# jwliao1209/DiffMusic

Hardware: AMD Instinct MI355X
Metric: denoising steps/sec (10 s clip, 200-step DPS) (higher is better)
Workload: dtype f16; 1 GPU; MusicLDM + DPS music_inpainting, 10 s @16 kHz, 200-step schedule, batch 8 per GPU (BASELINE.json configs[1]); global_batch=8, clips_per_gpu=8, lanes=1, parallelism=clip-sharded x1 (RCCL world size 1, no per-step collective), finite=True, nan_steps=0, settle_steps=10, cached_reference_transform=True, launched_by=single process

## Files before the change

diffmusic_amd/csrc/elementwise.hip:

```cpp
#include "dmx_common.h"
#include <cstdlib>
#include "kernels.h"

namespace {

__device__ __forceinline__ void unpack8(const uint4& u, float* f) {
  f[0] = alo(u.x); f[1] = ahi(u.x); f[2] = alo(u.y); f[3] = ahi(u.y);
  f[4] = alo(u.z); f[5] = ahi(u.z); f[6] = alo(u.w); f[7] = ahi(u.w);
}
__device__ __forceinline__ uint4 pack8(const float* f) {
  return make_uint4(pack2a(f[0], f[1]), pack2a(f[2], f[3]), pack2a(f[4], f[5]), pack2a(f[6], f[7]));
}
__device__ __forceinline__ float silu_f(float z) { return z / (1.f + __expf(-z)); }
__device__ __forceinline__ float dsilu_f(float z) {
  const float s = 1.f / (1.f + __expf(-z));
  return s * (1.f + z * (1.f - s));
}

template <int MODE>
__global__ void gn_partial_kernel(const act_t* __restrict__ x, const act_t* __restrict__ dy,
                                  const float* __restrict__ scale, const float* __restrict__ shift,
                                  const float* __restrict__ stats, float* __restrict__ partial,
                                  int P, int C, int G, int rpb, int ppb, int silu) {
  extern __shared__ float sh[];
// ... 967 lines not shown
}

__global__ void gather_col_f32_kernel(const float* __restrict__ x, float* __restrict__ y, long long rows, int ld, int col) {
  const long long idx = (long long)blockIdx.x * blockDim.x + threadIdx.x;
  if (idx < rows) y[idx] = x[idx * ld + col];
}
__global__ void tanh_bwd_pad8_kernel(const float* __restrict__ dwav, const float* __restrict__ wav8, act_t* __restrict__ gz,
                                     long long rows) {
  const long long idx = (long long)blockIdx.x * blockDim.x + threadIdx.x;
  if (idx >= rows) return;
  const float w = wav8[idx * 8];
  const float g = dwav[idx] * (1.f - w * w);
  reinterpret_cast<uint4*>(gz)[idx] = make_uint4((uint32_t)f2a(g), 0u, 0u, 0u);
}
__global__ void gather_col_f32_dead_kernel(const float* __restrict__ x, float* __restrict__ y, long long rows, int ld, int col, int T, int s0,
                                           int s1) {
  const long long idx = (long long)blockIdx.x * blockDim.x + threadIdx.x;
  if (idx >= rows) return;
  const int t = (int)(idx % T);
  y[idx] = (t >= s0 && t < s1) ? 0.f : x[idx * ld + col];
}
__global__ void tanh_bwd_pad8_dead_kernel(const float* __restrict__ dwav, const float* __restrict__ wav8, act_t* __restrict__ gz,
                                          long long rows, int T, int s0, int s1) {
  const long long idx = (long long)blockIdx.x * blockDim.x + threadIdx.x;
  if (idx >= rows) return;
  const int t = (int)(idx % T);
  float g = 0.f;
  if (!(t >= s0 && t < s1)) {
    const float w = wav8[idx * 8];
    g = dwav[idx] * (1.f - w * w);
  }
  reinterpret_cast<uint4*>(gz)[idx] = make_uint4((uint32_t)f2a(g), 0u, 0u, 0u);
}
__global__ void scatter_col_pad8_kernel(const float* __restrict__ v, act_t* __restrict__ y, long long rows, float scale) {
  const long long idx = (long long)blockIdx.x * blockDim.x + threadIdx.x;
  if (idx >= rows) return;
  reinterpret_cast<uint4*>(y)[idx] = make_uint4((uint32_t)f2a(v[idx] * scale), 0u, 0u, 0u);
}

__global__ void gather_col_f32_to_act_kernel(const float* __restrict__ x, act_t* __restrict__ y, long long rows, int ld, int col) {
  const long long idx = (long long)blockIdx.x * blockDim.x + threadIdx.x;
  if (idx < rows) y[idx] = f2a(x[idx * ld + col]);
}
__global__ void pad_col8_act_kernel(const act_t* __restrict__ v, act_t* __restrict__ y, long long rows) {
  const long long idx = (long long)blockIdx.x * blockDim.x + threadIdx.x;
  if (idx >= rows) return;
  reinterpret_cast<uint4*>(y)[idx] = make_uint4((uint32_t)v[idx], 0u, 0u, 0u);
}

constexpr int GN_SMALL_MAXU = 16;
__global__ __launch_bounds__(256) void gn_small_kernel(const act_t* __restrict__ x, act_t* __restrict__ y,
                                                       const float* __restrict__ gamma, const float* __restrict__ beta,
                                                       float* __restrict__ stats, float* __restrict__ scale, float* __restrict__ shift,
                                                       int P, int C, int G, float eps, int silu) {
  __shared__ float sh[16];
  const int g = blockIdx.x, b = blockIdx.y, cpg = C / G, U = cpg >> 2, c0 = g * cpg;
  const int units = P * U;
  const act_t* xb = x + (long long)b * P * C + c0;
  uint2 v[GN_SMALL_MAXU];
  float sum = 0.f;
#pragma unroll
  for (int i = 0; i < GN_SMALL_MAXU; ++i) {
    const int u = threadIdx.x + i * 256;
    v[i] = make_uint2(0, 0);
    if (u < units) {
      const int px = u / U, cu = u - px * U;
// ... 247 lines not shown
  hipLaunchKernelGGL(bf16_to_f32_kernel, dim3((unsigned)((n + 255) / 256)), dim3(256), 0, st, x, y, n, scale);
  return CHECK_LAUNCH();
}
int dmx_extract_col(const act_t* x, float* y, long long rows, int ld, int col, hipStream_t st) {
  hipLaunchKernelGGL(extract_col_kernel, dim3((unsigned)((rows + 255) / 256)), dim3(256), 0, st, x, y, rows, ld, col);
  return CHECK_LAUNCH();
}
int dmx_timestep_embed(const float* t, act_t* y, int B, int dim, hipStream_t st) {
  hipLaunchKernelGGL(timestep_embed_kernel, dim3(cdiv(B * dim, 256)), dim3(256), 0, st, t, y, B, dim);
  return CHECK_LAUNCH();
}

int dmx_gather_col_f32(const float* x, float* y, long long rows, int ld, int col, hipStream_t st) {
  hipLaunchKernelGGL(gather_col_f32_kernel, dim3((unsigned)((rows + 255) / 256)), dim3(256), 0, st, x, y, rows, ld, col);
  return CHECK_LAUNCH();
}
int dmx_tanh_bwd_pad8(const float* dwav, const float* wav8, act_t* gz, long long rows, hipStream_t st) {
  hipLaunchKernelGGL(tanh_bwd_pad8_kernel, dim3((unsigned)((rows + 255) / 256)), dim3(256), 0, st, dwav, wav8, gz, rows);
  return CHECK_LAUNCH();
}
int dmx_scatter_col_pad8(const float* v, act_t* y, long long rows, float scale, hipStream_t st) {
  hipLaunchKernelGGL(scatter_col_pad8_kernel, dim3((unsigned)((rows + 255) / 256)), dim3(256), 0, st, v, y, rows, scale);
  return CHECK_LAUNCH();
}

int dmx_gather_col_f32_dead(const float* x, float* y, long long rows, int ld, int col, int T, int s0, int s1, hipStream_t st) {
  hipLaunchKernelGGL(gather_col_f32_dead_kernel, dim3((unsigned)((rows + 255) / 256)), dim3(256), 0, st, x, y, rows, ld, col, T, s0, s1);
  return CHECK_LAUNCH();
}
int dmx_tanh_bwd_pad8_dead(const float* dwav, const float* wav8, act_t* gz, long long rows, int T, int s0, int s1, hipStream_t st) {
  hipLaunchKernelGGL(tanh_bwd_pad8_dead_kernel, dim3((unsigned)((rows + 255) / 256)), dim3(256), 0, st, dwav, wav8, gz, rows, T, s0, s1);
  return CHECK_LAUNCH();
}
int dmx_gather_col_f32_to_act(const float* x, act_t* y, long long rows, int ld, int col, hipStream_t st) {
  hipLaunchKernelGGL(gather_col_f32_to_act_kernel, dim3((unsigned)((rows + 255) / 256)), dim3(256), 0, st, x, y, rows, ld, col);
  return CHECK_LAUNCH();
}
int dmx_pad_col8_act(const act_t* v, act_t* y, long long rows, hipStream_t st) {
  hipLaunchKernelGGL(pad_col8_act_kernel, dim3((unsigned)((rows + 255) / 256)), dim3(256), 0, st, v, y, rows);
  return CHECK_LAUNCH();
}
```

diffmusic_amd/csrc/hifigan.hip:

```cpp
#include "models.h"
#include "conv_pair.h"
#include <cstdlib>

struct SplitKScope {
  explicit SplitKScope(float* ws, size_t bytes, bool on) : on_(on && ws) { if (on_) dmx_gemm_set_splitk_workspace(ws, bytes); }
  ~SplitKScope() { if (on_) dmx_gemm_set_splitk_workspace(nullptr, 0); }
  bool on_;
};

struct Span { int a = 0, b = 0; bool empty() const { return b <= a; } };
static inline Span span_meet(Span x, Span y) { Span r{x.a > y.a ? x.a : y.a, x.b < y.b ? x.b : y.b}; if (r.empty()) r = Span{}; return r; }
static inline long long floor_div(long long a, long long b) { return a >= 0 ? a / b : -((-a + b - 1) / b); }
static inline long long ceil_div(long long a, long long b) { return -floor_div(-a, b); }

int dmx_conv_dead_rows_impl(int k, int dil, int pad, int stride, int transposed, int t_in, int t_out, int a, int b, int* lo, int* hi) {
  *lo = *hi = 0;
  if (k < 1 || dil < 1 || stride < 1 || pad < 0 || t_in < 1 || t_out < 1) return DMX_ERR_SHAPE;
  if (!transposed && stride != 1) return DMX_ERR_SHAPE;
  if (a < 0) a = 0;
  if (b > t_out) b = t_out;
  if (b <= a) return DMX_OK;
  const long long INF = 1ll << 40;
  const long long ea = a == 0 ? -INF : a, eb = b == t_out ? INF : b;
  long long l, h;
// ... 195 lines not shown

  int out_len(int T_) const {
    int t = T_;
    for (int i = 0; i < ns; ++i) t = conv_out_len(ups[i], t);
    return t;
  }

  int forward(const act_t* mel, float* wav, int B_, int T_, void* ws, size_t ws_bytes, hipStream_t st, int s0 = 0, int s1 = 0) {
    if (cfg.model_in_dim & 7) return DMX_ERR_SHAPE;
    dry = (ws == nullptr);
    B = B_;
    if (!dry) {
      use_dead = false;
      if (s1 > s0) { make_plan(T_, s0, s1); use_dead = plan.on; }
    }
    const bool dead = use_dead && !dry;
    SplitKScope sk_scope(splitk_ws, kSplitKBytes, !dry && !multi_wanted());
    arena.reset(ws, dry ? (size_t)-1 : ws_bytes);
    T = T_;
    Ts.assign(ns, 0);
    xs_a.assign(ns, nullptr); act_out.assign(ns, nullptr);
    ha.assign(ns * nk * nd, nullptr); xa.assign(ns * nk * nd, nullptr);
    hb.assign(ns * nk * nd, nullptr); xb.assign(ns * nk * nd, nullptr);
    fused.assign(ns * nk * nd, 0);
    const float slope = cfg.leaky_relu_slope;
    auto bits = [&](size_t rows, int C) { return (unsigned char*)arena.raw(rows * (size_t)(C >> 3)); };
    act_pre = arena.bf((size_t)B * T * conv_pre.Cop);
    {
      Epi e; e.flags = EPI_LRELU2 | EPI_NO_C; e.act_slope = slope; e.C2 = act_pre;
      RUN(conv_fwd_1d(conv_pre, mel, act_pre, B, T, e, st));
    }
    const act_t* cur_act = act_pre;
    int Tin = T;
    for (int s = 0; s < ns; ++s) {
      const ConvLayer& up = ups[s];
      const int To = conv_out_len(up, Tin), C = up.Cop;
      const size_t n = (size_t)B * To * C;
      Ts[s] = To;
      xs_a[s] = arena.bf(n);
      act_out[s] = arena.bf(n);
      unsigned char* xs_b = nullptr;
      for (int k = 0; k < nk; ++k)
        for (int d = 0; d < nd; ++d) {
          const int id = idx(s, k, d);
          fused[id] = step_is_fused(id, To) ? 1 : 0;
          xa[id] = d == 0 ? xs_a[s] : arena.bf(n);
          if (fused[id]) {
            hb[id] = bits((size_t)B * To, C);
            if (d == 0) { if (!xs_b) xs_b = bits((size_t)B * To, C); xb[id] = xs_b; }
            else xb[id] = bits((size_t)B * To, C);
          } else {
            ha[id] = arena.bf(n);
          }
        }
      const size_t mk = arena.mark();
      act_t* sum = arena.bf(n);
      {
        Epi e; e.flags = EPI_LRELU2 | EPI_NO_C; e.act_slope = slope; e.C2 = xs_a[s];
        if (xs_b) { e.flags |= EPI_BITS2; e.B2 = xs_b; }
        RUN(conv_fwd_1d(up, cur_act, xs_a[s], B, Tin, e, st));
      }
      const float next_slope = (s == ns - 1) ? 0.01f : slope;
      const bool mt = multi();
      bool all_fused = nk <= 3;
      for (int k = 0; k < nk; ++k) for (int d = 0; d < nd; ++d) all_fused = all_fused && fused[idx(s, k, d)] != 0;
      if (all_fused && !mt) {
        for (int d = 0; d < nd; ++d) {
          GemmDesc da[DMX_MAX_STAGES], db[DMX_MAX_STAGES];
          const GemmDesc* pa[DMX_MAX_STAGES]; const GemmDesc* pb[DMX_MAX_STAGES];
          PairDead pd[DMX_MAX_STAGES];
          for (int k = 0; k < nk; ++k) {
            const int id = idx(s, k, d);
            if (dead) pd[k] = dead_fwd(id);
            {
              Epi e; e.flags = EPI_LRELU2 | EPI_NO_C | EPI_BITS2; e.act_slope = slope; e.B2 = hb[id];
              RUN(conv_fwd_1d_desc(c1[id], xa[id], ha[id], B, To, e, da[k]));
            }
            if (d < nd - 1) {
              const int idn = idx(s, k, d + 1);
              act_t* xn = xa[idn];
              Epi e; e.flags = EPI_RESID | EPI_RESID_INV | EPI_LRELU2 | EPI_NO_C | EPI_BITS2; e.R = xa[id]; e.resid_inv_slope = 1.f / slope;
              e.act_slope = slope; e.C2 = xn; e.B2 = xb[idn];
              RUN(conv_fwd_1d_desc(c2[id], ha[id], xn, B, To, e, db[k]));
            } else {
              Epi e; e.flags = EPI_RESID | EPI_RESID_INV; e.R = xa[id]; e.resid_inv_slope = 1.f / slope; e.alpha = 1.f / nk;
              if (k > 0) e.flags |= EPI_ACCUM;
              if (k == nk - 1) { e.flags |= EPI_LRELU2 | EPI_NO_C; e.act_slope = next_slope; e.C2 = act_out[s]; }
              RUN(conv_fwd_1d_desc(c2[id], ha[id], sum, B, To, e, db[k]));
            }
            pa[k] = &da[k]; pb[k] = &db[k];
          }
          if (dry) continue;
          for (int k = 0; k < nk; ++k)
            if (!dmx_conv_pair_eligible(&da[k], db[k])) {
              dmx_set_error("hifigan: resblock step %d was planned as fused but the pair kernel refuses it", idx(s, k, d));
              return DMX_ERR_STATE;
            }
          if (d < nd - 1) RUN(dmx_conv_pair_group_launch(nk, pa, pb, st, dead ? pd : nullptr));
          else for (int k = 0; k < nk; ++k) RUN(conv_pair_run(da[k], db[k], st, dead ? &pd[k] : nullptr));
        }
        arena.release(mk);
        cur_act = act_out[s];
        Tin = To;
        continue;
      }
      hipEvent_t fin_prev = nullptr;
      if (mt) {
        hipEvent_t e0 = next_event();
        (void)hipEventRecord(e0, st);
        for (int k = 1; k < nk; ++k) (void)hipStreamWaitEvent(bstream[k], e0, 0);
      }
      for (int k = 0; k < nk; ++k) {
        hipStream_t sk = (mt && k > 0) ? bstream[k] : st;
        for (int d = 0; d < nd; ++d) {
          const int id = idx(s, k, d);
          const bool fz = fused[id] != 0;
          GemmDesc da, db;
          {
            Epi e; e.flags = EPI_LRELU2 | EPI_NO_C; e.act_slope = slope;
            if (fz) { e.flags |= EPI_BITS2; e.B2 = hb[id]; } else e.C2 = ha[id];
            RUN(conv_fwd_1d_desc(c1[id], xa[id], ha[id], B, To, e, da));
          }
          if (d < nd - 1) {
            const int idn = idx(s, k, d + 1);
            act_t* xn = xa[idn];
            Epi e; e.flags = EPI_RESID | EPI_RESID_INV | EPI_LRELU2 | EPI_NO_C; e.R = xa[id]; e.resid_inv_slope = 1.f / slope;
            e.act_slope = slope; e.C2 = xn;
            if (fused[idn]) { e.flags |= EPI_BITS2; e.B2 = xb[idn]; }
            RUN(conv_fwd_1d_desc(c2[id], ha[id], xn, B, To, e, db));
          } else {
            Epi e; e.flags = EPI_RESID | EPI_RESID_INV; e.R = xa[id]; e.resid_inv_slope = 1.f / slope; e.alpha = 1.f / nk;
            if (k > 0) e.flags |= EPI_ACCUM;
            if (k == nk - 1) { e.flags |= EPI_LRELU2 | EPI_NO_C; e.act_slope = next_slope; e.C2 = act_out[s]; }
            RUN(conv_fwd_1d_desc(c2[id], ha[id], sum, B, To, e, db));
          }
          if (!dry && fz && !dmx_conv_pair_eligible(&da, db)) {
            dmx_set_error("hifigan: resblock step %d was planned as fused but the pair kernel refuses it", id);
            return DMX_ERR_STATE;
          }
          if (d == nd - 1 && mt && fin_prev) (void)hipStreamWaitEvent(sk, fin_prev, 0);
          RUN(conv_pair_run(da, db, sk));
          if (d == nd - 1 && mt) { fin_prev = next_event(); (void)hipEventRecord(fin_prev, sk); }
        }
      }
      if (mt && fin_prev) (void)hipStreamWaitEvent(st, fin_prev, 0);
      arena.release(mk);
      cur_act = act_out[s];
      Tin = To;
    }
    const int Tout = Tin;
    wav8 = arena.f32((size_t)B * Tout * 8);
    CHECK_WS("hifigan");
    {
      Epi e; e.flags = EPI_F32OUT | EPI_TANH;
      RUN(conv_fwd_1d(conv_post, cur_act, wav8, B, Tout, e, st));
    }
    if (dead) RUN(dmx_gather_col_f32_dead(wav8, wav, (long long)B * Tout, 8, 0, Tout, plan.wav.a, plan.wav.b, st));
    else RUN(dmx_gather_col_f32(wav8, wav, (long long)B * Tout, 8, 0, st));
    have_tape = true;
    return DMX_OK;
  }

  int backward(const float* dwav, act_t* dmel, hipStream_t st) {
    if (!have_tape && !dry) { dmx_set_error("hifigan backward without forward"); return DMX_ERR_STATE; }
    SplitKScope sk_scope(splitk_ws, kSplitKBytes, !dry && !multi_wanted());
    const float slope = cfg.leaky_relu_slope;
    const int Tout = Ts[ns - 1];
    const size_t mk0 = arena.mark();
    act_t* gz = arena.bf((size_t)B * Tout * 8);
    const int Clast = ups[ns - 1].Cop;
    act_t* g = arena.bf((size_t)B * Tout * Clast);
    CHECK_WS("hifigan");
    const bool dead = use_dead && !dry;
    if (dead) RUN(dmx_tanh_bwd_pad8_dead(dwav, wav8, gz, (long long)B * Tout, Tout, plan.wav.a, plan.wav.b, st));
    else RUN(dmx_tanh_bwd_pad8(dwav, wav8, gz, (long long)B * Tout, st));
    {
      Epi e; e.flags = EPI_MASK; e.X = act_out[ns - 1]; e.mask_slope = 0.01f; e.alpha = 1.f / nk;
      RUN(conv_bwd_1d(conv_post, gz, g, B, Tout, e, st));
    }
    for (int s = ns - 1; s >= 0; --s) {
      const int To = Ts[s], Tin = s == 0 ? T : Ts[s - 1], C = ups[s].Cop;
      const size_t n = (size_t)B * To * C;
      act_t* gxs = arena.bf(n);
      act_t* ghk[DMX_MAX_STAGES];
      act_t* gAB[DMX_MAX_STAGES][2];
      for (int k = 0; k < nk; ++k) { ghk[k] = arena.bf(n); gAB[k][0] = arena.bf(n); gAB[k][1] = arena.bf(n); }
      const int Cin = ups[s].Cip;
      act_t* gprev = arena.bf((size_t)B * Tin * Cin);
      CHECK_WS("hifigan");
      const bool mt = multi();
      hipEvent_t fin_prev = nullptr;
      bool all_fused = nk <= 3;
      for (int k = 0; k < nk; ++k) for (int d = 0; d < nd; ++d) all_fused = all_fused && fused[idx(s, k, d)] != 0;
      if (all_fused && !mt) {
        const act_t* gcs[DMX_MAX_STAGES];
        for (int k = 0; k < nk; ++k) gcs[k] = g;
        if (dead && !plan.xs[s].empty() &&
            hipMemset2DAsync(gxs + (size_t)plan.xs[s].a * C, (size_t)To * C * sizeof(act_t), 0, (size_t)(plan.xs[s].b - plan.xs[s].a) * C * sizeof(act_t),
                             (size_t)B, st) != hipSuccess) {
          dmx_set_error("hifigan: clearing the dead rows of a stage gradient failed");
          return DMX_ERR_LAUNCH;
        }
        for (int d = nd - 1; d >= 0; --d) {
          GemmDesc da[DMX_MAX_STAGES], db[DMX_MAX_STAGES];
          const GemmDesc* pa[DMX_MAX_STAGES]; const GemmDesc* pb[DMX_MAX_STAGES];
          act_t* dsts[DMX_MAX_STAGES];
          PairDead pd[DMX_MAX_STAGES];
          for (int k = 0; k < nk; ++k) {
            const int id = idx(s, k, d);
            if (dead) pd[k] = dead_bwd(s, id, d);
            {
              Epi e; e.mask_slope = slope; e.flags = EPI_MASKBITS; e.XB = hb[id];
              RUN(conv_bwd_1d_desc(c2[id], gcs[k], ghk[k], B, To, e, da[k]));
            }
            Epi e; e.flags = EPI_RESID | EPI_MASKBITS; e.mask_slope = slope; e.R = gcs[k]; e.XB = xb[id];
            if (d == 0) { dsts[k] = gxs; if (k > 0) e.flags |= EPI_ACCUM; }
            else dsts[k] = (gcs[k] == gAB[k][0]) ? gAB[k][1] : gAB[k][0];
            RUN(conv_bwd_1d_desc(c1[id], ghk[k], dsts[k], B, To, e, db[k]));
            pa[k] = &da[k]; pb[k] = &db[k];
          }
          if (!dry) {
            if (d > 0) RUN(dmx_conv_pair_group_launch(nk, pa, pb, st, dead ? pd : nullptr));
            else for (int k = 0; k < nk; ++k) RUN(conv_pair_run(da[k], db[k], st, dead ? &pd[k] : nullptr));
          }
          for (int k = 0; k < nk; ++k) gcs[k] = dsts[k];
        }
      } else {
      if (mt) {
        hipEvent_t e0 = next_event();
        (void)hipEventRecord(e0, st);
        for (int k = 1; k < nk; ++k) (void)hipStreamWaitEvent(bstream[k], e0, 0);
      }
      for (int k = 0; k < nk; ++k) {
        hipStream_t sk = (mt && k > 0) ? bstream[k] : st;
        const act_t* gc = g;
// ... 74 lines not shown
```

diffmusic_amd/csrc/kernels.h:

```cpp
#pragma once
#include "dmx_common.h"

#define DMX_GN_MAX_CHUNKS 512

size_t dmx_gn_scratch_floats(int B, int C, int G);
struct GnRegion {
  float* part = nullptr;
  int tm = 0, P = 0, nq = 0;
  int qoff = 0, cq = 0;
};
struct GnParts { int n = 0; GnRegion r[8]; };
size_t dmx_gn_part_floats(int B, int P, int N);
int dmx_groupnorm_fwd(const act_t* x, act_t* y, const float* gamma, const float* beta, float* stats, float* scale,
                      float* shift, float* partial, int B, int P, int C, int G, float eps, int silu, hipStream_t st,
                      const GnParts* parts = nullptr);
int dmx_groupnorm_bwd(const act_t* x, const act_t* dy, const act_t* add, act_t* dx, const float* stats,
                      const float* scale, const float* shift, float* k0, float* k1, float* partial, int B, int P, int C,
                      int G, int silu, hipStream_t st, const GnParts* parts = nullptr);
int dmx_layernorm_fwd(const act_t* x, act_t* y, const float* gamma, const float* beta, int rows, int C, float eps,
                      hipStream_t st);
int dmx_softmax_fwd(const float* S, act_t* P, const float* colbias, long long rows, int N, long long lds, long long ldp,
                    int rows_per_bias, hipStream_t st);
int dmx_softmax_act(const act_t* S, act_t* P, const float* colbias, long long rows, int N, long long ldp, int rows_per_bias,
                    hipStream_t st);
int dmx_rowdot(const act_t* a, const act_t* b, float* out, long long rows, int C, long long lda, long long ldb, hipStream_t st);
int dmx_geglu(const act_t* x, act_t* y, long long rows, int I, hipStream_t st);
int dmx_silu(const act_t* x, act_t* y, long long n, hipStream_t st);
int dmx_upsample_nearest(const act_t* x, act_t* y, int B, int Hi, int Wi, int Ho, int Wo, int C, hipStream_t st);
int dmx_upsample2x_bwd(const act_t* dy, act_t* dx, int B, int Hi, int Wi, int C, hipStream_t st);
int dmx_transpose(const act_t* in, act_t* out, int R, int C, long long ldi, long long ldo, int Z, int Zi, long long sIo,
                  long long sIi, long long sOo, long long sOi, hipStream_t st);
int dmx_concat2(const act_t* a, const act_t* b, act_t* dst, long long rows, int Ca, int Cb, hipStream_t st);
int dmx_copy_channels(const act_t* src, act_t* dst, long long rows, int C, int lds, int ldd, int soff, int doff,
                      hipStream_t st);
int dmx_axpby(const act_t* x, const act_t* y0, act_t* y, float a, float b, long long n, hipStream_t st);
int dmx_nchw_f32_to_nhwc_bf16(const float* x, act_t* y, int B, int C, int HW, int Cp, float scale, hipStream_t st);
int dmx_nhwc_bf16_to_nchw_f32(const act_t* x, float* y, int B, int C, int HW, int Cp, float scale, hipStream_t st);
int dmx_f32_to_bf16(const float* x, act_t* y, long long n, float scale, hipStream_t st);
int dmx_bf16_to_f32(const act_t* x, float* y, long long n, float scale, hipStream_t st);
int dmx_extract_col(const act_t* x, float* y, long long rows, int ld, int col, hipStream_t st);
int dmx_gather_col_f32(const float* x, float* y, long long rows, int ld, int col, hipStream_t st);
int dmx_tanh_bwd_pad8(const float* dwav, const float* wav8, act_t* gz, long long rows, hipStream_t st);
int dmx_gather_col_f32_dead(const float* x, float* y, long long rows, int ld, int col, int T, int s0, int s1, hipStream_t st);
int dmx_tanh_bwd_pad8_dead(const float* dwav, const float* wav8, act_t* gz, long long rows, int T, int s0, int s1, hipStream_t st);
int dmx_scatter_col_pad8(const float* v, act_t* y, long long rows, float scale, hipStream_t st);
int dmx_gather_col_f32_to_act(const float* x, act_t* y, long long rows, int ld, int col, hipStream_t st);
int dmx_pad_col8_act(const act_t* v, act_t* y, long long rows, hipStream_t st);
int dmx_timestep_embed(const float* t, act_t* y, int B, int dim, hipStream_t st);

bool dmx_flash_attn_ok(int dh, int C);
int dmx_flash_attn_fwd(const act_t* q, const act_t* k, const act_t* v, act_t* o, const float* colbias, int B, int Nq, int Nk,
                       int C, int heads, float scale, hipStream_t st, int ldq = 0, int ldk = 0, int ldv = 0, int* qt_out = nullptr);

int dmx_stft_tables(float* table, float* tableT, int n_fft, int bins, int Npad, int Kpad, int hann, hipStream_t st);
int dmx_stft_fwd(const float* wav, long long wav_stride, const float* table, float* X, int B, int L, int T, int n_fft, int hop, int Npad,
                 hipStream_t st);
int dmx_stft_bwd_frames(const float* Y, const float* tableT, float* dframe, int M, int n_fft, int Kpad, hipStream_t st);
int dmx_mel_fwd(const float* X, const float* fb, float* mel_lin, float* mel_out, int rows, int ldx, int bins, int n_mels, int power2,
                int to_db, float lo, float hi, hipStream_t st);
int dmx_mel_bwd(const float* X, const float* fb, const float* mel_lin, const float* dmel, float* Y, int rows, int ldx, int ldy, int bins,
                int n_mels, int power2, int to_db, float lo, float hi, hipStream_t st);
int dmx_stft_mag(const float* X, float* mag, int B, int T, int bins, int ldx, hipStream_t st);
int dmx_stft_mag_bwd(const float* X, const float* dmag, float* Y, int B, int T, int bins, int ldx, int ldy, hipStream_t st);
int dmx_overlap_add(const float* dframe, float* dwav, long long out_stride, int B, int T, int L, int n_fft, int hop, int accumulate,
                    hipStream_t st);
int dmx_l2_loss_grad(const float* ref, const float* pred, float* loss, float* dpred, int B, long long n, long long ref_stride, float gscale,
                     hipStream_t st);
int dmx_mask_mul(const float* x, long long xs, const float* mask, float* y, long long ys, int B, int L, int Ly, hipStream_t st);
int dmx_melscale(const float* mag, const float* fb, float* mel, int B, int T, int bins, int n_mels, float lo, float hi, hipStream_t st);
int dmx_absmax_normalize(float* x, float* inv_scale, int B, long long n, float target, hipStream_t st);

struct DmxStftMelTables {
  const float2* tw;
  const float* win;
  const int *klo, *klen; const float* fbc; int kmax;
  const int *mlo, *mlen; const float* fbr; int mmax;
};
// ... 28 lines not shown
```

diffmusic_amd/csrc/layers.h:

```cpp
#pragma once
#include <string>
#include <vector>
#include <map>
#include <cstdio>
#include <cstring>
#include "dmx_common.h"
#include "kernels.h"

void dmx_set_error(const char* fmt, ...);

inline int pad8(int c) { return (c + 7) & ~7; }

struct Arena {
  char* base = nullptr;
  size_t cap = 0, off = 0, peak = 0;
  bool overflow = false;
  void reset(void* b, size_t c) { base = (char*)b; cap = c; off = 0; overflow = false; }
  void* raw(size_t bytes) {
    bytes = align_up(bytes, 256);
    if (off + bytes > cap) { overflow = true; off += bytes; if (off > peak) peak = off; return base; }
    void* p = base + off;
    off += bytes;
    if (off > peak) peak = off;
    return p;
// ... 9 lines not shown
  std::vector<int> shape;
  size_t numel = 0;
  float* dev = nullptr;
  bool loaded = false;
};

struct ParamStore {
  std::vector<Param> params;
  std::map<std::string, int> index;
  std::vector<void*> owned;
  int add(const std::string& name, std::vector<int> shape);
  float* dev(int id) const { return params[id].dev; }
  int load(const char* name, const float* host, size_t numel);
  bool all_loaded(std::string* missing) const;
  void* dalloc(size_t bytes);
  void free_all();
};

struct ConvLayer {
  int Ci = 0, Co = 0, Cip = 0, Cop = 0;
  int kh = 1, kw = 1, stride = 1, dil = 1, pad_h = 0, pad_w = 0;
  int pad_h_hi = 0, pad_w_hi = 0;
  bool transposed = false;
  bool has_bias = true, need_bwd = false;
  bool geglu = false;
  int w_id = -1, b_id = -1;
  int ln_g_id = -1, ln_b_id = -1;
  float ln_eps = 1e-5f;
  float* colsum = nullptr;
  std::vector<act_t*> wf;
  std::vector<std::vector<int>> wf_taps;
  act_t* wb = nullptr;
  float* bias = nullptr;
  std::vector<act_t*> wup;
  act_t* wup_b = nullptr;
  int ntaps() const { return kh * kw; }
};

struct Epi {
  int flags = 0;
  float alpha = 1.f, act_slope = 0.f, mask_slope = 0.f, resid_inv_slope = 1.f;
  const act_t* R = nullptr;
  const act_t* X = nullptr;
  act_t* C2 = nullptr;
  const float* rowbias = nullptr;
  int ldrb = 0;
  const unsigned char* XB = nullptr;
  unsigned char* B2 = nullptr;
  float* rowstats_out = nullptr;
  const float* rowstats_in = nullptr;
  int nslots = 0;
  float* gn_part = nullptr;
  const act_t* gnb_x = nullptr;
  const float* gnb_scale = nullptr;
  const float* gnb_shift = nullptr;
  int gnb_silu = 0, gnb_cpg = 0;
  const float* gnb_stats = nullptr;
};

ConvLayer make_conv1d(ParamStore& ps, const std::string& prefix, int Ci, int Co, int k, int dil, int pad, bool need_bwd);
ConvLayer make_convT1d(ParamStore& ps, const std::string& prefix, int Ci, int Co, int k, int stride, int pad, bool need_bwd);
ConvLayer make_conv2d(ParamStore& ps, const std::string& prefix, int Ci, int Co, int k, int stride, int pad, bool need_bwd);
ConvLayer make_conv2d_asym(ParamStore& ps, const std::string& prefix, int Ci, int Co, int k, int stride, int pad_lo, int pad_hi);
ConvLayer make_linear(ParamStore& ps, const std::string& prefix, int Ci, int Co, bool bias, bool need_bwd);
int pack_layer(ParamStore& ps, ConvLayer& L, hipStream_t st);
int pack_linear_stack(ParamStore& ps, ConvLayer& dst, const ConvLayer* const* src, int n, hipStream_t st);

int conv_out_len(const ConvLayer& L, int Ti);
int conv_fwd_1d(const ConvLayer& L, const act_t* in, void* out, int B, int Ti, const Epi& e, hipStream_t st);
int conv_bwd_1d(const ConvLayer& L, const act_t* dout, void* din, int B, int Ti, const Epi& e, hipStream_t st);
int conv_fwd_1d_desc(const ConvLayer& L, const act_t* in, void* out, int B, int Ti, const Epi& e, GemmDesc& d);
int conv_bwd_1d_desc(const ConvLayer& L, const act_t* dout, void* din, int B, int Ti, const Epi& e, GemmDesc& d);
struct PairDead;
int conv_pair_run(const GemmDesc& a, const GemmDesc& b, hipStream_t st, const PairDead* dead = nullptr);
int conv_fwd_2d(const ConvLayer& L, const act_t* in, void* out, int B, int Hi, int Wi, const Epi& e, hipStream_t st, int* gn_rows = nullptr);
int pack_layer_up2x(ParamStore& ps, ConvLayer& L, hipStream_t st);
int conv_up2x_fwd(const ConvLayer& L, const act_t* in, void* out, int B, int Hi, int Wi, const Epi& e, hipStream_t st,
                  float* const* gn_buf = nullptr, int* gn_rows = nullptr);
int conv_up2x_bwd(const ConvLayer& L, const act_t* dout, void* din, int B, int Hi, int Wi, const Epi& e, hipStream_t st);
int conv_bwd_2d(const ConvLayer& L, const act_t* dout, void* din, int B, int Hi, int Wi, const Epi& e, hipStream_t st, int* gn_rows = nullptr);
struct GemmBatch { int Z = 1, Zi = 1; long long sAo = 0, sAi = 0, sBo = 0, sBi = 0, sCo = 0, sCi = 0; };
int gemm_nt(const act_t* A, int lda, const act_t* Bm, int ldb, void* C, int ldc, int M, int N, int K, const Epi& e,
            const GemmBatch& gb, hipStream_t st);
int linear_fwd(const ConvLayer& L, const act_t* in, int lda, void* out, int ldc, long long rows, const Epi& e, hipStream_t st);
int linear_bwd(const ConvLayer& L, const act_t* dout, int lda, void* din, int ldc, long long rows, const Epi& e, hipStream_t st);

struct GroupNormLayer {
  int C = 0, G = 32, g_id = -1, b_id = -1;
  float eps = 1e-5f;
};
GroupNormLayer make_gn(ParamStore& ps, const std::string& prefix, int C, int G, float eps);
struct GnSave { float* stats = nullptr; float* scale = nullptr; float* shift = nullptr; };
```

diffmusic_amd/csrc/layers.hip:

```cpp
#include "layers.h"
#include "conv_pair.h"
#include <cstdarg>

static thread_local char g_err[512] = "";
void dmx_set_error(const char* fmt, ...) {
  va_list ap;
  va_start(ap, fmt);
  vsnprintf(g_err, sizeof(g_err), fmt, ap);
  va_end(ap);
}
extern "C" const char* dmx_last_error() { return g_err; }

int ParamStore::add(const std::string& name, std::vector<int> shape) {
  Param p;
  p.name = name;
  p.shape = shape;
  p.numel = 1;
  for (int s : shape) p.numel *= (size_t)s;
  p.dev = (float*)dalloc(p.numel * sizeof(float));
  index[name] = (int)params.size();
  params.push_back(p);
  return (int)params.size() - 1;
}
void* ParamStore::dalloc(size_t bytes) {
// ... 193 lines not shown
  const int T = L.ntaps();
  if (T > DMX_MAX_TAPS) { dmx_set_error("too many taps"); return DMX_ERR_SHAPE; }
  std::vector<int> all(T);
  for (int i = 0; i < T; ++i) all[i] = i;
  int gh = 0;
  if (L.geglu) {
    if (L.transposed || T != 1 || L.need_bwd || (L.Co & 31) || L.Cop != L.Co) { dmx_set_error("GEGLU packing needs a forward-only linear layer with Cout %% 32 == 0"); return DMX_ERR_SHAPE; }
    gh = L.Co / 2;
  }
  float* ln_w = nullptr;
  float* ln_bias = nullptr;
  if (L.ln_g_id >= 0) {
    if (L.transposed || T != 1 || L.need_bwd) { dmx_set_error("LayerNorm fold needs a forward-only linear layer"); return DMX_ERR_SHAPE; }
    if (hipMalloc(&ln_w, (size_t)L.Co * L.Ci * sizeof(float)) != hipSuccess) return DMX_ERR_PARAM;
    ln_bias = (float*)ps.dalloc((size_t)L.Co * sizeof(float));
    if (!ln_bias) { (void)hipFree(ln_w); return DMX_ERR_PARAM; }
    hipLaunchKernelGGL(ln_fold_kernel, dim3(L.Co), dim3(256), 0, st, w, ps.dev(L.ln_g_id), ps.dev(L.ln_b_id),
                       L.has_bias ? ps.dev(L.b_id) : (const float*)nullptr, ln_w, ln_bias, L.Ci);
    w = ln_w;
  }
  if (!L.transposed) {
    L.wf.push_back(pack(ps, w, L.Cop, L.Co, T, L.Cip, L.Ci, (long long)L.Ci * T, T, 1, all, st, gh));
    if (L.need_bwd) L.wb = pack(ps, w, L.Cip, L.Ci, T, L.Cop, L.Co, T, (long long)L.Ci * T, 1, all, st);
  } else {
    const int k = L.kw, s = L.stride, p = L.pad_w;
    for (int r = 0; r < s; ++r) {
      const int j0 = (r + p) % s;
      std::vector<int> taps;
      for (int j = j0; j < k; j += s) taps.push_back(j);
      L.wf_taps.push_back(taps);
      L.wf.push_back(pack(ps, w, L.Cop, L.Co, (int)taps.size(), L.Cip, L.Ci, k, (long long)L.Co * k, 1, taps, st));
    }
    if (L.need_bwd) L.wb = pack(ps, w, L.Cip, L.Ci, k, L.Cop, L.Co, (long long)L.Co * k, k, 1, all, st);
  }
  L.bias = (float*)ps.dalloc(L.Cop * sizeof(float));
  hipLaunchKernelGGL(pad_bias_kernel, dim3(cdiv(L.Cop, 256)), dim3(256), 0, st,
                     ln_bias ? (const float*)ln_bias : (L.has_bias ? ps.dev(L.b_id) : (const float*)nullptr), L.bias, L.Co, L.Cop, gh);
  for (act_t* pw : L.wf) if (!pw) { if (ln_w) (void)hipFree(ln_w); return DMX_ERR_PARAM; }
  if (ln_w) {
    L.has_bias = true;
    L.colsum = (float*)ps.dalloc(L.Cop * sizeof(float));
    if (!L.colsum) { (void)hipFree(ln_w); return DMX_ERR_PARAM; }
    hipLaunchKernelGGL(packed_rowsum_kernel, dim3(L.Cop), dim3(64), 0, st, L.wf[0], L.colsum, L.Cip);
    (void)hipStreamSynchronize(st);
    (void)hipFree(ln_w);
  }
  return hipGetLastError() == hipSuccess ? DMX_OK : DMX_ERR_LAUNCH;
}

int pack_linear_stack(ParamStore& ps, ConvLayer& dst, const ConvLayer* const* src, int n, hipStream_t st) {
  if (n < 1) return DMX_ERR_SHAPE;
  const int Ci = src[0]->Ci;
  int Co = 0;
  bool bias = false, bwd = false;
  for (int i = 0; i < n; ++i) {
    if (src[i]->Ci != Ci || src[i]->ntaps() != 1 || src[i]->transposed) { dmx_set_error("stacked projection: linear layers of equal input width"); return DMX_ERR_SHAPE; }
    Co += src[i]->Co; bias = bias || src[i]->has_bias; bwd = bwd || src[i]->need_bwd;
  }
  float *w = nullptr, *b = nullptr;
  if (hipMalloc(&w, (size_t)Co * Ci * sizeof(float)) != hipSuccess || hipMalloc(&b, (size_t)Co * sizeof(float)) != hipSuccess) {
    if (w) (void)hipFree(w);
    return DMX_ERR_PARAM;
  }
  (void)hipMemsetAsync(b, 0, (size_t)Co * sizeof(float), st);
  size_t off = 0;
  for (int i = 0; i < n; ++i) {
    (void)hipMemcpyAsync(w + off * Ci, ps.dev(src[i]->w_id), (size_t)src[i]->Co * Ci * sizeof(float), hipMemcpyDeviceToDevice, st);
    if (src[i]->has_bias) (void)hipMemcpyAsync(b + off, ps.dev(src[i]->b_id), (size_t)src[i]->Co * sizeof(float), hipMemcpyDeviceToDevice, st);
    off += src[i]->Co;
  }
// ... 46 lines not shown
}
int conv_fwd_1d_desc(const ConvLayer& L, const act_t* in, void* out, int B, int Ti, const Epi& e, GemmDesc& d) {
  if (L.transposed) return DMX_ERR_SHAPE;
  const int To = conv_out_len(L, Ti);
  fwd_1d_common(d, L, in, out, Ti, To, e);
  d.W = L.wf[0]; d.ntaps = L.kw; d.K = L.kw * L.Cip; d.ldw = d.K;
  d.Hq = 1; d.Wq = To; d.sx = L.stride; d.M = B * To;
  for (int t = 0; t < L.kw; ++t) { d.tdy[t] = 0; d.tdx[t] = (signed char)(t * L.dil - L.pad_w); }
  return DMX_OK;
}

int conv_fwd_1d(const ConvLayer& L, const act_t* in, void* out, int B, int Ti, const Epi& e, hipStream_t st) {
  const int To = conv_out_len(L, Ti);
  GemmDesc d;
  if (!L.transposed) {
    const int rc = conv_fwd_1d_desc(L, in, out, B, Ti, e, d);
    return rc != DMX_OK ? rc : dmx_gemm_launch(d, st);
  }
  fwd_1d_common(d, L, in, out, Ti, To, e);
  const int s = L.stride, p = L.pad_w;
  for (int r = 0; r < s; ++r) {
    GemmDesc q = d;
    const int nt = (int)L.wf_taps[r].size();
    const int base = (r + p) / s;
    q.W = L.wf[r]; q.ntaps = nt; q.K = nt * L.Cip; q.ldw = q.K;
    q.Hq = 1; q.Wq = cdiv(To - r, s); q.M = B * q.Wq;
    q.osx = s; q.oox = r;
    for (int i = 0; i < nt; ++i) { q.tdy[i] = 0; q.tdx[i] = (signed char)(base - i); }
    if (q.Wq <= 0) continue;
    const int rc = dmx_gemm_launch(q, st);
    if (rc != DMX_OK) return rc;
  }
  return DMX_OK;
}

int conv_bwd_1d_desc(const ConvLayer& L, const act_t* dout, void* din, int B, int Ti, const Epi& e, GemmDesc& d) {
  if (!L.wb) { dmx_set_error("layer has no dgrad weights"); return DMX_ERR_STATE; }
  const int To = conv_out_len(L, Ti);
  init_desc(d, e);
  d.A = dout; d.Hi = 1; d.Wi = To; d.Ci = L.Cop; d.lda = L.Cop;
  d.W = L.wb; d.ntaps = L.kw; d.K = L.kw * L.Cop; d.ldw = d.K;
  d.N = L.Cip;
  d.Hq = 1; d.Wq = Ti; d.M = B * Ti;
  set_out(d, din, 1, Ti, L.Cip);
  if (!L.transposed) {
    if (L.stride != 1) return DMX_ERR_SHAPE;
    for (int t = 0; t < L.kw; ++t) { d.tdy[t] = 0; d.tdx[t] = (signed char)(L.pad_w - t * L.dil); }
  } else {
    d.sx = L.stride;
    for (int t = 0; t < L.kw; ++t) { d.tdy[t] = 0; d.tdx[t] = (signed char)(t - L.pad_w); }
  }
  return DMX_OK;
}
int conv_bwd_1d(const ConvLayer& L, const act_t* dout, void* din, int B, int Ti, const Epi& e, hipStream_t st) {
  GemmDesc d;
  const int rc = conv_bwd_1d_desc(L, dout, din, B, Ti, e, d);
  return rc != DMX_OK ? rc : dmx_gemm_launch(d, st);
}

int conv_pair_run(const GemmDesc& a, const GemmDesc& b, hipStream_t st, const PairDead* dead) {
  if (dmx_conv_pair_eligible(&a, b)) return dmx_conv_pair_launch(&a, b, st, dead);
  if (dead) { dmx_set_error("conv_pair_run: dead rows need the fused pair kernel"); return DMX_ERR_SHAPE; }
  const int rc = dmx_gemm_launch(a, st);
  return rc != DMX_OK ? rc : dmx_gemm_launch(b, st);
}

// ... 120 lines not shown
```

Before: 27.05 steps/s (weak scaling: one step advances a batch of 8 clips on one GPU; value = K / wall x 1 GPU(s)).

## Merge transposed-conv phases into one GEMM and batch dead-row gradient clears

For HiFi-GAN upsampling transposed convolutions with k-2p==s, the weights of all stride phases are repacked into one zero-padded union-tap weight, so the forward pass runs a single GEMM with N=stride*Cout instead of one GEMM per phase. The output layout [Ti, s*C] matches the interleaved [s*Ti, C] layout, so no scatter is needed. The aim is fewer launches and better tile use, at the cost of extra FLOPs on the zero-padded taps. Separately, the per-stage hipMemset2DAsync calls that clear dead gradient rows are replaced by one batched fill kernel launched before the backward loop.

```diff
diff --git a/diffmusic_amd/csrc/elementwise.hip b/diffmusic_amd/csrc/elementwise.hip
--- a/diffmusic_amd/csrc/elementwise.hip
+++ b/diffmusic_amd/csrc/elementwise.hip
@@ -1023,6 +1023,14 @@
   }
   reinterpret_cast<uint4*>(gz)[idx] = make_uint4((uint32_t)f2a(g), 0u, 0u, 0u);
 }
+__global__ void fill_rows_zero_kernel(const FillRowsArgs a) {
+  const FillRows f = a.r[blockIdx.y];
+  const long long per_row = f.row_bytes >> 4, total = per_row * f.rows;
+  for (long long i = (long long)blockIdx.x * blockDim.x + threadIdx.x; i < total; i += (long long)gridDim.x * blockDim.x) {
+    const long long r = i / per_row, c = i - r * per_row;
+    *reinterpret_cast<uint4*>(f.base + r * f.pitch + c * 16) = make_uint4(0u, 0u, 0u, 0u);
+  }
+}
 __global__ void scatter_col_pad8_kernel(const float* __restrict__ v, act_t* __restrict__ y, long long rows, float scale) {
   const long long idx = (long long)blockIdx.x * blockDim.x + threadIdx.x;
   if (idx >= rows) return;
@@ -1336,6 +1344,25 @@
   hipLaunchKernelGGL(tanh_bwd_pad8_dead_kernel, dim3((unsigned)((rows + 255) / 256)), dim3(256), 0, st, dwav, wav8, gz, rows, T, s0, s1);
   return CHECK_LAUNCH();
 }
+int dmx_fill_rows_zero(const FillRows* ranges, int n, hipStream_t st) {
+  if (n < 0 || n > DMX_FILL_MAX) return DMX_ERR_SHAPE;
+  FillRowsArgs a;
+  int m = 0;
+  long long most = 0;
+  for (int i = 0; i < n; ++i) {
+    const FillRows& f = ranges[i];
+    if (f.rows <= 0 || f.row_bytes <= 0) continue;
+    if (!f.base || ((size_t)f.base & 15) || (f.pitch & 15) || (f.row_bytes & 15) || f.pitch < f.row_bytes) return DMX_ERR_SHAPE;
+    a.r[m++] = f;
+    const long long q = (f.row_bytes >> 4) * f.rows;
+    if (q > most) most = q;
+  }
+  if (m == 0) return DMX_OK;
+  for (int i = m; i < DMX_FILL_MAX; ++i) a.r[i] = FillRows{nullptr, 0, 0, 0};
+  const long long blocks = (most + 255) / 256;
+  hipLaunchKernelGGL(fill_rows_zero_kernel, dim3((unsigned)(blocks < 2048 ? blocks : 2048), (unsigned)m), dim3(256), 0, st, a);
+  return CHECK_LAUNCH();
+}
 int dmx_gather_col_f32_to_act(const float* x, act_t* y, long long rows, int ld, int col, hipStream_t st) {
   hipLaunchKernelGGL(gather_col_f32_to_act_kernel, dim3((unsigned)((rows + 255) / 256)), dim3(256), 0, st, x, y, rows, ld, col);
   return CHECK_LAUNCH();
diff --git a/diffmusic_amd/csrc/hifigan.hip b/diffmusic_amd/csrc/hifigan.hip
--- a/diffmusic_amd/csrc/hifigan.hip
+++ b/diffmusic_amd/csrc/hifigan.hip
@@ -251,6 +251,7 @@
     }
     const act_t* cur_act = act_pre;
     int Tin = T;
+    bool in_rows_complete = true;
     for (int s = 0; s < ns; ++s) {
       const ConvLayer& up = ups[s];
       const int To = conv_out_len(up, Tin), C = up.Cop;
@@ -277,7 +278,10 @@
       {
         Epi e; e.flags = EPI_LRELU2 | EPI_NO_C; e.act_slope = slope; e.C2 = xs_a[s];
         if (xs_b) { e.flags |= EPI_BITS2; e.B2 = xs_b; }
-        RUN(conv_fwd_1d(up, cur_act, xs_a[s], B, Tin, e, st));
+        static const bool ups_phases = getenv("DMX_UPS_PHASES") != nullptr;
+        const bool merged = !ups_phases && in_rows_complete && (long long)B * Tin > 8192 && conv_fwd_1d_can_merge(up, Tin);
+        if (merged) RUN(conv_fwd_1d_merged(up, cur_act, xs_a[s], B, Tin, e, st));
+        else RUN(conv_fwd_1d(up, cur_act, xs_a[s], B, Tin, e, st));
       }
       const float next_slope = (s == ns - 1) ? 0.01f : slope;
       const bool mt = multi();
@@ -321,6 +325,7 @@
         arena.release(mk);
         cur_act = act_out[s];
         Tin = To;
+        in_rows_complete = false;
         continue;
       }
       hipEvent_t fin_prev = nullptr;
@@ -366,6 +371,7 @@
       arena.release(mk);
       cur_act = act_out[s];
       Tin = To;
+      in_rows_complete = true;
     }
     const int Tout = Tin;
     wav8 = arena.f32((size_t)B * Tout * 8);
@@ -397,6 +403,30 @@
       Epi e; e.flags = EPI_MASK; e.X = act_out[ns - 1]; e.mask_slope = 0.01f; e.alpha = 1.f / nk;
       RUN(conv_bwd_1d(conv_post, gz, g, B, Tout, e, st));
     }
+    auto grouped_stage = [&](int s) {
+      bool all = nk <= 3;
+      for (int k = 0; k < nk; ++k) for (int d = 0; d < nd; ++d) all = all && fused[idx(s, k, d)] != 0;
+      return all && !multi();
+    };
+    if (dead) {
+      static_assert(DMX_FILL_MAX >= DMX_MAX_STAGES, "one fill range per stage");
+      FillRows fr[DMX_MAX_STAGES];
+      int nf = 0;
+      const size_t mk1 = arena.mark();
+      for (int s = ns - 1; s >= 0; --s) {
+        const int To = Ts[s], Tin = s == 0 ? T : Ts[s - 1], C = ups[s].Cop;
+        const size_t n = (size_t)B * To * C;
+        act_t* gxs = arena.bf(n);
+        for (int k = 0; k < 3 * nk; ++k) (void)arena.bf(n);
+        (void)arena.bf((size_t)B * Tin * ups[s].Cip);
+        if (grouped_stage(s) && !plan.xs[s].empty())
+          fr[nf++] = FillRows{(char*)(gxs + (size_t)plan.xs[s].a * C), (long long)To * C * (long long)sizeof(act_t),
+                              (long long)(plan.xs[s].b - plan.xs[s].a) * C * (long long)sizeof(act_t), B};
+      }
+      CHECK_WS("hifigan");
+      arena.release(mk1);
+      RUN(dmx_fill_rows_zero(fr, nf, st));
+    }
     for (int s = ns - 1; s >= 0; --s) {
       const int To = Ts[s], Tin = s == 0 ? T : Ts[s - 1], C = ups[s].Cop;
       const size_t n = (size_t)B * To * C;
@@ -409,17 +439,9 @@
       CHECK_WS("hifigan");
       const bool mt = multi();
       hipEvent_t fin_prev = nullptr;
-      bool all_fused = nk <= 3;
-      for (int k = 0; k < nk; ++k) for (int d = 0; d < nd; ++d) all_fused = all_fused && fused[idx(s, k, d)] != 0;
-      if (all_fused && !mt) {
+      if (grouped_stage(s)) {
         const act_t* gcs[DMX_MAX_STAGES];
         for (int k = 0; k < nk; ++k) gcs[k] = g;
-        if (dead && !plan.xs[s].empty() &&
-            hipMemset2DAsync(gxs + (size_t)plan.xs[s].a * C, (size_t)To * C * sizeof(act_t), 0, (size_t)(plan.xs[s].b - plan.xs[s].a) * C * sizeof(act_t),
-                             (size_t)B, st) != hipSuccess) {
-          dmx_set_error("hifigan: clearing the dead rows of a stage gradient failed");
-          return DMX_ERR_LAUNCH;
-        }
         for (int d = nd - 1; d >= 0; --d) {
           GemmDesc da[DMX_MAX_STAGES], db[DMX_MAX_STAGES];
           const GemmDesc* pa[DMX_MAX_STAGES]; const GemmDesc* pb[DMX_MAX_STAGES];
diff --git a/diffmusic_amd/csrc/kernels.h b/diffmusic_amd/csrc/kernels.h
--- a/diffmusic_amd/csrc/kernels.h
+++ b/diffmusic_amd/csrc/kernels.h
@@ -43,6 +43,10 @@
 int dmx_tanh_bwd_pad8(const float* dwav, const float* wav8, act_t* gz, long long rows, hipStream_t st);
 int dmx_gather_col_f32_dead(const float* x, float* y, long long rows, int ld, int col, int T, int s0, int s1, hipStream_t st);
 int dmx_tanh_bwd_pad8_dead(const float* dwav, const float* wav8, act_t* gz, long long rows, int T, int s0, int s1, hipStream_t st);
+struct FillRows { char* base; long long pitch, row_bytes; int rows; };
+constexpr int DMX_FILL_MAX = 8;
+struct FillRowsArgs { FillRows r[DMX_FILL_MAX]; };
+int dmx_fill_rows_zero(const FillRows* ranges, int n, hipStream_t st);
 int dmx_scatter_col_pad8(const float* v, act_t* y, long long rows, float scale, hipStream_t st);
 int dmx_gather_col_f32_to_act(const float* x, act_t* y, long long rows, int ld, int col, hipStream_t st);
 int dmx_pad_col8_act(const act_t* v, act_t* y, long long rows, hipStream_t st);
diff --git a/diffmusic_amd/csrc/layers.h b/diffmusic_amd/csrc/layers.h
--- a/diffmusic_amd/csrc/layers.h
+++ b/diffmusic_amd/csrc/layers.h
@@ -65,6 +65,9 @@
   std::vector<std::vector<int>> wf_taps;
   act_t* wb = nullptr;
   float* bias = nullptr;
+  act_t* wm = nullptr;
+  float* bias_m = nullptr;
+  int wm_taps = 0, wm_off0 = 0;
   std::vector<act_t*> wup;
   act_t* wup_b = nullptr;
   int ntaps() const { return kh * kw; }
@@ -102,6 +105,8 @@
 int conv_out_len(const ConvLayer& L, int Ti);
 int conv_fwd_1d(const ConvLayer& L, const act_t* in, void* out, int B, int Ti, const Epi& e, hipStream_t st);
 int conv_bwd_1d(const ConvLayer& L, const act_t* dout, void* din, int B, int Ti, const Epi& e, hipStream_t st);
+bool conv_fwd_1d_can_merge(const ConvLayer& L, int Ti);
+int conv_fwd_1d_merged(const ConvLayer& L, const act_t* in, void* out, int B, int Ti, const Epi& e, hipStream_t st);
 int conv_fwd_1d_desc(const ConvLayer& L, const act_t* in, void* out, int B, int Ti, const Epi& e, GemmDesc& d);
 int conv_bwd_1d_desc(const ConvLayer& L, const act_t* dout, void* din, int B, int Ti, const Epi& e, GemmDesc& d);
 struct PairDead;
diff --git a/diffmusic_amd/csrc/layers.hip b/diffmusic_amd/csrc/layers.hip
--- a/diffmusic_amd/csrc/layers.hip
+++ b/diffmusic_amd/csrc/layers.hip
@@ -249,10 +249,37 @@
       L.wf.push_back(pack(ps, w, L.Cop, L.Co, (int)taps.size(), L.Cip, L.Ci, k, (long long)L.Co * k, 1, taps, st));
     }
     if (L.need_bwd) L.wb = pack(ps, w, L.Cip, L.Ci, k, L.Cop, L.Co, (long long)L.Co * k, k, 1, all, st);
+    int omax = -(1 << 30), omin = 1 << 30;
+    bool every_phase_has_taps = true;
+    for (int r = 0; r < s; ++r) {
+      const int base = (r + p) / s, nt = (int)L.wf_taps[r].size();
+      if (nt < 1) { every_phase_has_taps = false; break; }
+      omax = base > omax ? base : omax;
+      omin = base - (nt - 1) < omin ? base - (nt - 1) : omin;
+    }
+    const int U = omax - omin + 1;
+    if (s > 1 && k - 2 * p == s && every_phase_has_taps && U <= DMX_MAX_TAPS && omax <= 127 && omin >= -128) {
+      const long long blk = (long long)L.Cop * U * L.Cip;
+      L.wm = (act_t*)ps.dalloc((size_t)blk * s * 2);
+      L.bias_m = (float*)ps.dalloc((size_t)s * L.Cop * sizeof(float));
+      if (!L.wm || !L.bias_m) return DMX_ERR_PARAM;
+      for (int r = 0; r < s; ++r) {
+        const int base = (r + p) / s;
+        PackTaps pt;
+        for (int i = 0; i < DMX_MAX_TAPS; ++i) pt.idx[i] = -1;
+        for (int i = 0; i < (int)L.wf_taps[r].size(); ++i) pt.idx[omax - (base - i)] = L.wf_taps[r][i];
+        hipLaunchKernelGGL(pack_weight_kernel, dim3((unsigned)((blk + 255) / 256)), dim3(256), 0, st, w, L.wm + blk * r, L.Cop, L.Co, U, L.Cip,
+                           L.Ci, (long long)k, (long long)L.Co * k, 1ll, pt, 0);
+      }
+      L.wm_taps = U; L.wm_off0 = omax;
+    }
   }
   L.bias = (float*)ps.dalloc(L.Cop * sizeof(float));
   hipLaunchKernelGGL(pad_bias_kernel, dim3(cdiv(L.Cop, 256)), dim3(256), 0, st,
                      ln_bias ? (const float*)ln_bias : (L.has_bias ? ps.dev(L.b_id) : (const float*)nullptr), L.bias, L.Co, L.Cop, gh);
+  if (L.wm)
+    for (int r = 0; r < L.stride; ++r)
+      (void)hipMemcpyAsync(L.bias_m + (size_t)r * L.Cop, L.bias, L.Cop * sizeof(float), hipMemcpyDeviceToDevice, st);
   for (act_t* pw : L.wf) if (!pw) { if (ln_w) (void)hipFree(ln_w); return DMX_ERR_PARAM; }
   if (ln_w) {
     L.has_bias = true;
@@ -365,6 +392,24 @@
     if (rc != DMX_OK) return rc;
   }
   return DMX_OK;
+}
+
+bool conv_fwd_1d_can_merge(const ConvLayer& L, int Ti) {
+  return L.transposed && L.wm && L.bias_m && conv_out_len(L, Ti) == L.stride * Ti && !(L.Cip & 31);
+}
+int conv_fwd_1d_merged(const ConvLayer& L, const act_t* in, void* out, int B, int Ti, const Epi& e, hipStream_t st) {
+  if (!conv_fwd_1d_can_merge(L, Ti)) { dmx_set_error("conv_fwd_1d_merged: layer has no merged form at this length"); return DMX_ERR_SHAPE; }
+  const int N = L.stride * L.Cop, U = L.wm_taps;
+  GemmDesc d;
+  init_desc(d, e);
+  if (L.has_bias) { d.bias = L.bias_m; d.flags |= EPI_BIAS; }
+  d.A = in; d.Hi = 1; d.Wi = Ti; d.Ci = L.Cip; d.lda = L.Cip;
+  d.N = N;
+  set_out(d, out, 1, Ti, N);
+  d.W = L.wm; d.ntaps = U; d.K = U * L.Cip; d.ldw = d.K;
+  d.Hq = 1; d.Wq = Ti; d.M = B * Ti;
+  for (int u = 0; u < U; ++u) { d.tdy[u] = 0; d.tdx[u] = (signed char)(L.wm_off0 - u); }
+  return dmx_gemm_launch(d, st);
 }
 
 int conv_bwd_1d_desc(const ConvLayer& L, const act_t* dout, void* din, int B, int Ti, const Epi& e, GemmDesc& d) {
```

Result: no change. 27.18 steps/s (weak scaling: one step advances a batch of 8 clips on one GPU; value = K / wall x 1 GPU(s)) (median of 6 runs) (+0.5%).
